# evroon/mav-detection

Measured on NVIDIA B200. Metric: 1080p frame-pairs/sec (flow+FoE+mask), higher is better.
Workload: dtype f32

## Files before the change

### include/mavd.h

```cpp
#ifndef MAVD_H_
#define MAVD_H_

#include <stddef.h>
#include <stdint.h>

#ifdef __cplusplus
extern "C" {
#endif

#define MAVD_ABI_VERSION 3

enum {
    MAVD_OK = 0,
    MAVD_ERR_INVALID = 1,
    MAVD_ERR_CUDA = 2,
    MAVD_ERR_UNSUPPORTED = 3,
    MAVD_ERR_NOMEM = 4
};

#define MAVD_FARNEBACK_GAUSSIAN 256

#define MAVD_N_SAMPLE_PAIRS 1000
#define MAVD_SAMPLES_PER_FRAME (4 * MAVD_N_SAMPLE_PAIRS)
#define MAVD_MAX_BOXES 32
// ... 14 lines not shown
    int32_t device;
    int32_t width;
    int32_t height;
    int32_t max_pairs;
    mavd_farneback_params farneback;
} mavd_config;

typedef struct mavd_imu {
    double ang[3];
    double dt;
    int32_t derotate;
    int32_t _pad;
} mavd_imu;

typedef struct mavd_detect_params {
    double magnitude_threshold;
    double ransac_threshold;
    double dyn_offset;
    double dyn_base;
    double dyn_gain;
    double dyn_min_mag;
    double fixed_min_mag;
    double fixed_angle;
} mavd_detect_params;

typedef struct mavd_tuning {
    int32_t mat_coord;
    int32_t pyr_staged;
    int32_t use_graph;
    int32_t polyexp_tma;
    int32_t iter_small_tiles;
    int32_t use_pdl;
    int32_t pyr_sweep;
    int32_t reserved[1];
} mavd_tuning;

typedef struct mavd_aux_inputs {
    const uint8_t* sky; int64_t sky_stride;
    const uint8_t* seg; int64_t seg_stride;
    const float* gt_flow;
} mavd_aux_inputs;

#define MAVD_HOST_BGR 1
#define MAVD_HOST_SEG_PACKED 2
#define MAVD_HOST_SKY_PACKED 4
#define MAVD_HOST_FIXED_PACKED 8
#define MAVD_HOST_COPY_ONLY 16

typedef struct mavd_frame_stats {
    double max_phi;
    int64_t n_total;
    int64_t n_fixed;
    int64_t positives;
    int64_t negatives;
    int64_t tp_total, fp_total;
    int64_t tp_fixed, fp_fixed;
    int32_t seg_bbox[4];
    double seg_flow_sum[2];
    double gt_flow_sum[2];
} mavd_frame_stats;

typedef struct mavd_frame_record {
    double foe[2];
    int32_t n_intersections;
    int32_t n_labels;
    mavd_frame_stats stats;
    int32_t boxes[MAVD_MAX_BOXES][5];
// ... 174 lines not shown
```

### mav_detection_b200/_lib.py

```python
from __future__ import annotations

import ctypes as C
import os
from typing import Optional

_HERE = os.path.dirname(os.path.abspath(__file__))
LIB_PATH = os.path.join(_HERE, 'csrc', 'libmavd.so')

ABI_VERSION = 3
MAVD_OK, MAVD_ERR_INVALID, MAVD_ERR_CUDA, MAVD_ERR_UNSUPPORTED, MAVD_ERR_NOMEM = 0, 1, 2, 3, 4
N_SAMPLE_PAIRS = 1000
SAMPLES_PER_FRAME = 4 * N_SAMPLE_PAIRS
MAX_BOXES = 32
HOST_SLOTS = 3
MAX_DETECTIONS = 256
OPTFLOW_FARNEBACK_GAUSSIAN = 256


class FarnebackParams(C.Structure):
    _fields_ = [('pyr_scale', C.c_double), ('levels', C.c_int32), ('winsize', C.c_int32),
                ('iterations', C.c_int32), ('poly_n', C.c_int32), ('poly_sigma', C.c_double),
                ('flags', C.c_int32)]


# ... 2 lines not shown
                ('max_pairs', C.c_int32), ('farneback', FarnebackParams)]


class Imu(C.Structure):
    _fields_ = [('ang', C.c_double * 3), ('dt', C.c_double), ('derotate', C.c_int32), ('_pad', C.c_int32)]


class DetectParams(C.Structure):
    _fields_ = [('magnitude_threshold', C.c_double), ('ransac_threshold', C.c_double),
                ('dyn_offset', C.c_double), ('dyn_base', C.c_double), ('dyn_gain', C.c_double),
                ('dyn_min_mag', C.c_double), ('fixed_min_mag', C.c_double), ('fixed_angle', C.c_double)]


class FrameStats(C.Structure):
    _fields_ = [('max_phi', C.c_double), ('n_total', C.c_int64), ('n_fixed', C.c_int64),
                ('positives', C.c_int64), ('negatives', C.c_int64), ('tp_total', C.c_int64),
                ('fp_total', C.c_int64), ('tp_fixed', C.c_int64), ('fp_fixed', C.c_int64),
                ('seg_bbox', C.c_int32 * 4), ('seg_flow_sum', C.c_double * 2), ('gt_flow_sum', C.c_double * 2)]


class FrameRecord(C.Structure):
    _fields_ = [('foe', C.c_double * 2), ('n_intersections', C.c_int32), ('n_labels', C.c_int32),
                ('stats', FrameStats), ('boxes', (C.c_int32 * 5) * MAX_BOXES)]


class Detection(C.Structure):
    _fields_ = [('label', C.c_int32), ('box', C.c_int32 * 4), ('area', C.c_int32), ('sum_x', C.c_int64),
                ('sum_y', C.c_int64), ('flow_sum', C.c_double * 2)]


class Tuning(C.Structure):
    _fields_ = [('mat_coord', C.c_int32), ('pyr_staged', C.c_int32), ('use_graph', C.c_int32),
                ('polyexp_tma', C.c_int32), ('iter_small_tiles', C.c_int32), ('use_pdl', C.c_int32),
                ('pyr_sweep', C.c_int32), ('reserved', C.c_int32 * 1)]


class AuxInputs(C.Structure):
    _fields_ = [('sky', C.c_void_p), ('sky_stride', C.c_int64), ('seg', C.c_void_p), ('seg_stride', C.c_int64),
                ('gt_flow', C.c_void_p)]


HOST_BGR, HOST_SEG_PACKED, HOST_SKY_PACKED, HOST_FIXED_PACKED, HOST_COPY_ONLY = 1, 2, 4, 8, 16

PROF_CLASSES = 12
PROF_NAMES = ['pyramid', 'polyexp', 'matrices', 'iter_full', 'iter_full_last', 'iter_coarse', 'foe', 'residual',
              'ccl']


class Profile(C.Structure):
    _fields_ = [('ms', C.c_double * PROF_CLASSES), ('launches', C.c_int64 * PROF_CLASSES)]


_P = C.c_void_p
SIGNATURES = {
    'mavd_abi_version': (C.c_int, []),
    'mavd_last_error': (C.c_char_p, []),
    'mavd_default_detect_params': (None, [C.POINTER(DetectParams)]),
    'mavd_create': (C.c_int, [C.POINTER(Config), C.POINTER(_P)]),
    'mavd_destroy': (C.c_int, [_P]),
    'mavd_workspace_bytes': (C.c_int, [_P, C.POINTER(C.c_size_t)]),
    'mavd_default_tuning': (None, [C.POINTER(Tuning)]),
    'mavd_set_tuning': (C.c_int, [_P, C.POINTER(Tuning)]),
    'mavd_get_tuning': (C.c_int, [_P, C.POINTER(Tuning)]),
    'mavd_level_info': (C.c_int, [_P, C.POINTER(C.c_int32), C.POINTER(C.c_int32), C.POINTER(C.c_int32)]),
    'mavd_bgr2gray': (C.c_int, [_P, _P, C.c_int64, _P]),
    'mavd_farneback': (C.c_int, [_P, _P, C.c_int32, C.c_int32, _P, _P]),
    'mavd_farneback_tap': (C.c_int, [_P, C.c_int32, C.c_int32, C.c_int32, _P, _P]),
# ... 91 lines not shown
```

### mav_detection_b200/csrc/api.cu

```cuda
#include <math.h>
#include <stdarg.h>
#include <stdlib.h>
#include <string.h>

#include <algorithm>
#include <new>
#include <vector>

#include "common.cuh"

namespace mavd {

static thread_local char g_err[512] = "";
std::atomic<int64_t> g_launches{0};

void set_error(const char* fmt, ...) {
    va_list ap;
    va_start(ap, fmt);
    vsnprintf(g_err, sizeof(g_err), fmt, ap);
    va_end(ap);
}

static inline int cv_round(double v) { return (int)nearbyint(v); }

// ... 431 lines not shown
    }
    H->bytes = A.bytes;
    cudaError_t e = cudaDeviceSynchronize();
    if (e != cudaSuccess) {
        set_error("device error during create: %s", cudaGetErrorString(e));
        return fail(MAVD_ERR_CUDA);
    }
    *out = H;
    return MAVD_OK;
#undef C_TRY
}

int mavd_destroy(mavd_handle h) {
    if (!h) return MAVD_OK;
    mavd_handle_full* H = static_cast<mavd_handle_full*>(h);
    DeviceGuard dg(H->cfg.device);
    cudaDeviceSynchronize();
    for (void* p : H->arena.ptrs) cudaFree(p);
    release_host_side(H);
    delete H;
    return MAVD_OK;
}

void mavd_default_tuning(mavd_tuning* t) {
    if (!t) return;
    memset(t, 0, sizeof(*t));
    t->mat_coord = 0;
    t->pyr_staged = 1;
    t->use_graph = 1;
    t->polyexp_tma = 1;
    t->iter_small_tiles = 1;
    t->use_pdl = 1;
    t->pyr_sweep = 1;
}

int mavd_set_tuning(mavd_handle h, const mavd_tuning* t) {
    MAVD_REQUIRE(h && t, MAVD_ERR_INVALID, "set_tuning: NULL argument");
    MAVD_REQUIRE(t->mat_coord >= 0 && t->mat_coord <= 2, MAVD_ERR_INVALID, "set_tuning: value out of range");
    DeviceGuard dg(h->cfg.device);
    MAVD_CUDA(cudaDeviceSynchronize());
    drop_graphs(h);
    h->tune = *t;
    return MAVD_OK;
}

int mavd_graph_stats(mavd_handle h, int32_t* n_captured, int32_t* n_direct) {
    MAVD_REQUIRE(h && n_captured && n_direct, MAVD_ERR_INVALID, "graph_stats: NULL argument");
    *n_captured = *n_direct = 0;
    for (const auto& g : h->graphs) ++*(g.exec ? n_captured : n_direct);
    return MAVD_OK;
}

int mavd_get_tuning(mavd_handle h, mavd_tuning* out) {
    MAVD_REQUIRE(h && out, MAVD_ERR_INVALID, "get_tuning: NULL argument");
    *out = h->tune;
    return MAVD_OK;
}

int mavd_profile_enable(mavd_handle h, int32_t on) {
    MAVD_REQUIRE(h != nullptr, MAVD_ERR_INVALID, "profile: handle is NULL");
    DeviceGuard dg(h->cfg.device);
    MAVD_CUDA(cudaDeviceSynchronize());
    for (auto& r : h->prof.recs) { h->prof.pool.push_back(r.a); h->prof.pool.push_back(r.b); }
    h->prof.recs.clear();
    h->prof.on = on != 0;
    return MAVD_OK;
// ... 807 lines not shown
```

### mav_detection_b200/csrc/farneback.cu

```cuda
#include <math.h>

#include "common.cuh"

namespace mavd {

__device__ __forceinline__ int reflect101(int i, int n) {
    while (i < 0 || i >= n) {
        if (n == 1) return 0;
        i = (i < 0) ? -i : 2 * (n - 1) - i;
    }
    return i;
}

__device__ __forceinline__ int clampi(int v, int lo, int hi) { return v < lo ? lo : (v > hi ? hi : v); }

struct PyrLevel {
    int w, h, pitch, taps;
    const int* xbase; const float* xtab;
    const float* xtabT;
    int staged;
    const int* ybase; const float* ytab;
    float* tmp; float* img;
    size_t tmp_stride, img_stride;
    int row0;
    int htiles_x;
};
struct PyrDesc {
    int n;
    PyrLevel lv[kMaxLevels];
};

__device__ __forceinline__ float byte_to_float(uint32_t v, uint32_t selector) {
    return __uint_as_float(__byte_perm(v, 0x4B000000u, selector)) - 8388608.f;
// ... 504 lines not shown
                    for (int k = 0; k < 4; ++k) {
                        const int gx = clampi(gx0 + k, 0, w - 1);
                        const int xm = reflect101(gx - 1, w), xp = reflect101(gx + 1, w);
                        const float h0 = 0.25f * q0[xm] + 0.5f * q0[gx] + 0.25f * q0[xp];
                        const float h1 = 0.25f * q1[xm] + 0.5f * q1[gx] + 0.25f * q1[xp];
                        const float h2 = 0.25f * q2[xm] + 0.5f * q2[gx] + 0.25f * q2[xp];
                        o[k] = 0.25f * h0 + 0.5f * h1 + 0.25f * h2;
                    }
                    v = make_float4(o[0], o[1], o[2], o[3]);
                }
                *reinterpret_cast<float4*>(&raw[(rr + PE_H - n) * PE_RW + 4 * g]) = v;
            }
        }
    }
    __syncthreads();
    polyexp_passes<N_>(raw, t, pc, n, tid, x0, y0, h, pitch, R + (size_t)blockIdx.z * 5 * plane, plane);
}

__device__ __forceinline__ void st_global_f32(float* p, float v) {
    asm volatile("st.global.f32 [%0], %1;" ::"l"(p), "f"(v));
}

__device__ __forceinline__ float border_factor(int d) { return d < 2 ? 0.14f : 0.4472f; }

struct R0Px { float y, x, yy, xx, xy; };

__device__ __forceinline__ R0Px load_r0_px(const float* __restrict__ R0, size_t o, size_t plane) {
    R0Px r;
    r.y = __ldg(R0 + o); r.x = __ldg(R0 + plane + o); r.yy = __ldg(R0 + 2 * plane + o);
    r.xx = __ldg(R0 + 3 * plane + o); r.xy = __ldg(R0 + 4 * plane + o);
    return r;
}

__device__ __forceinline__ void update_matrices_px(int x, int y, int w, int h, int pitch, size_t plane, float dx,
                                                   float dy, const R0Px& r0,
                                                   const float* __restrict__ R1, float* __restrict__ Mout) {
    const size_t o = (size_t)y * pitch + x;
    const float r0y = r0.y, r0x = r0.x, r0yy = r0.yy, r0xx = r0.xx, r0xy = r0.xy;
    float fx = (float)x + dx, fy = (float)y + dy;
    const float flx = floorf(fx), fly = floorf(fy);
    const int x1 = (int)fminf(fmaxf(flx, -2.f), 1.0e6f), y1 = (int)fminf(fmaxf(fly, -2.f), 1.0e6f);
    fx -= flx;
    fy -= fly;
    float r2, r3, r4, r5, r6;
    if ((unsigned)x1 < (unsigned)(w - 1) && (unsigned)y1 < (unsigned)(h - 1)) {
        const float a00 = (1.f - fx) * (1.f - fy), a01 = fx * (1.f - fy), a10 = (1.f - fx) * fy, a11 = fx * fy;
        const float* p = R1 + (size_t)y1 * pitch + x1;
        r2 = a00 * __ldg(p) + a01 * __ldg(p + 1) + a10 * __ldg(p + pitch) + a11 * __ldg(p + pitch + 1);
        p += plane;
        r3 = a00 * __ldg(p) + a01 * __ldg(p + 1) + a10 * __ldg(p + pitch) + a11 * __ldg(p + pitch + 1);
        p += plane;
        r4 = a00 * __ldg(p) + a01 * __ldg(p + 1) + a10 * __ldg(p + pitch) + a11 * __ldg(p + pitch + 1);
        p += plane;
        r5 = a00 * __ldg(p) + a01 * __ldg(p + 1) + a10 * __ldg(p + pitch) + a11 * __ldg(p + pitch + 1);
        p += plane;
        r6 = a00 * __ldg(p) + a01 * __ldg(p + 1) + a10 * __ldg(p + pitch) + a11 * __ldg(p + pitch + 1);
        r4 = (r0yy + r4) * 0.5f;
        r5 = (r0xx + r5) * 0.5f;
        r6 = (r0xy + r6) * 0.25f;
    } else {
        r2 = r3 = 0.f;
        r4 = r0yy;
        r5 = r0xx;
        r6 = r0xy * 0.5f;
    }
    r2 = (r0y - r2) * 0.5f;
    r3 = (r0x - r3) * 0.5f;
    r2 += r4 * dy + r6 * dx;
    r3 += r6 * dy + r5 * dx;
    if ((unsigned)(x - 5) >= (unsigned)(w - 10) || (unsigned)(y - 5) >= (unsigned)(h - 10)) {
        const float sc = (x < 5 ? border_factor(x) : 1.f) * (x >= w - 5 ? border_factor(w - x - 1) : 1.f) *
                         (y < 5 ? border_factor(y) : 1.f) * (y >= h - 5 ? border_factor(h - y - 1) : 1.f);
        r2 *= sc; r3 *= sc; r4 *= sc; r5 *= sc; r6 *= sc;
    }
    Mout[o] = r4 * r4 + r6 * r6;
    Mout[plane + o] = (r4 + r5) * r6;
    Mout[2 * plane + o] = r5 * r5 + r6 * r6;
    Mout[3 * plane + o] = r4 * r2 + r6 * r3;
    Mout[4 * plane + o] = r6 * r2 + r5 * r3;
}

__device__ __forceinline__ void resize_coord(int d, double scale, int src, int& i0, float& a) {
    const float f = (float)__dsub_rn(__dmul_rn(__dadd_rn((double)d, 0.5), scale), 0.5);
    int s = (int)floorf(f);
    a = f - (float)s;
    if (s < 0) { s = 0; a = 0.f; }
    if (s >= src - 1) { s = src - 1; a = 0.f; }
    i0 = s;
}

enum { MI_COORD_F64 = 0, MI_COORD_TABLES = 1, MI_COORD_POW2 = 2 };

__device__ __forceinline__ void resize_coord_pow2(int d, float scale, int src, int& i0, float& a) {
    const float f = __fsub_rn(__fmul_rn(__fadd_rn((float)d, 0.5f), scale), 0.5f);
    int s = (int)floorf(f);
    a = f - (float)s;
    if (s < 0) { s = 0; a = 0.f; }
    if (s >= src - 1) { s = src - 1; a = 0.f; }
    i0 = s;
}

constexpr int MI_TX = 64, MI_TY = 4;

template <int COORD>
__global__ void __launch_bounds__(256, 8) matrices_init_kernel(const float* __restrict__ R, size_t plane, int w, int h,
                                                           int pitch, size_t R_pair_stride,
                                                           const float2* __restrict__ cflow, int cw, int ch,
                                                           int cpitch, size_t cflow_stride,
                                                           const int* __restrict__ fxi0,
                                                           const float* __restrict__ fxa,
                                                           const int* __restrict__ fyi0,
                                                           const float* __restrict__ fya, float up_scale,
                                                           float* __restrict__ M, double xscale, double yscale, int r0_first) {
    pdl_entry();
    const int p = blockIdx.x;
    const int x = blockIdx.y * MI_TX + (threadIdx.x & (MI_TX - 1));
    const int y = blockIdx.z * MI_TY + threadIdx.x / MI_TX;
    if (x >= w || y >= h) return;
    const float* R0 = R + (size_t)p * R_pair_stride;
    R0Px r0;
    if (r0_first) r0 = load_r0_px(R0, (size_t)y * pitch + x, plane);
    float dx = 0.f, dy = 0.f;
    if (cflow) {
        const float2* cf = cflow + (size_t)p * cflow_stride;
        int xa0, ya0;
        float ax, ay;
        if (COORD == MI_COORD_TABLES) {
            xa0 = fxi0[x]; ya0 = fyi0[y]; ax = fxa[x]; ay = fya[y];
        } else if (COORD == MI_COORD_POW2) {
            resize_coord_pow2(x, (float)xscale, cw, xa0, ax);
            resize_coord_pow2(y, (float)yscale, ch, ya0, ay);
        } else {
            resize_coord(x, xscale, cw, xa0, ax);
            resize_coord(y, yscale, ch, ya0, ay);
        }
        const int xa1 = min(xa0 + 1, cw - 1), ya1 = min(ya0 + 1, ch - 1);
        const float2 f00 = cf[(size_t)ya0 * cpitch + xa0], f01 = cf[(size_t)ya0 * cpitch + xa1];
        const float2 f10 = cf[(size_t)ya1 * cpitch + xa0], f11 = cf[(size_t)ya1 * cpitch + xa1];
        const float tx0 = f00.x * (1.f - ax) + f01.x * ax, tx1 = f10.x * (1.f - ax) + f11.x * ax;
        const float ty0 = f00.y * (1.f - ax) + f01.y * ax, ty1 = f10.y * (1.f - ax) + f11.y * ax;
        dx = (tx0 * (1.f - ay) + tx1 * ay) * up_scale;
        dy = (ty0 * (1.f - ay) + ty1 * ay) * up_scale;
    }
    if (!r0_first) r0 = load_r0_px(R0, (size_t)y * pitch + x, plane);
    update_matrices_px(x, y, w, h, pitch, plane, dx, dy, r0, R0 + 5 * plane, M + (size_t)p * 5 * plane);
}

constexpr int IT_TX = 64, IT_TY = 32;
constexpr int IT_PAIR_GROUP = 4;

struct IterArgs {
    const float* Min;
    float* Mout;
    const float* R;
    float2* flow;
    int flow_pitch;
    size_t flow_stride;
    int w, h, pitch;
    size_t plane;
    int m;
    int hx;
    float scale;
    int pair_stride;
    const float* gk;
    int n_pairs, tiles_x;
};

template <int M_>
__device__ __forceinline__ void hsum_box(const float (&u)[20], float (&o)[4]) {
    float s = 0.f;
#pragma unroll
    for (int j = 8 - M_; j <= 8 + M_; ++j) s += u[j];
    o[0] = s;
#pragma unroll
    for (int j = 1; j < 4; ++j) {
        s += u[8 + M_ + j] - u[8 - M_ + j - 1];
        o[j] = s;
    }
}

template <int M_>
__device__ __forceinline__ void hsum_gauss(const float (&u)[20], const float* __restrict__ gk, float (&o)[4]) {
    float k[M_ + 1];
#pragma unroll
    for (int i = 0; i <= M_; ++i) k[i] = gk[i];
#pragma unroll
    for (int j = 0; j < 4; ++j) {
        float s = __fmul_rn(u[8 + j], k[0]);
#pragma unroll
        for (int i = 1; i <= M_; ++i) s = __fmaf_rn(u[8 + j - i] + u[8 + j + i], k[i], s);
        o[j] = s;
    }
}

template <int M_>
__device__ __forceinline__ void hsum_gauss_reg(const float (&u)[20], const float (&k)[M_ + 1], float (&o)[4]) {
#pragma unroll
    for (int j = 0; j < 4; ++j) {
// ... 297 lines not shown
                 a10 * __ldg(R1 + (q1 + plane)) + a11 * __ldg(R1 + (q1 + plane) + 1);
            r4 = a00 * __ldg(R1 + (q0 + 2 * plane)) + a01 * __ldg(R1 + (q0 + 2 * plane) + 1) +
                 a10 * __ldg(R1 + (q1 + 2 * plane)) + a11 * __ldg(R1 + (q1 + 2 * plane) + 1);
            r5 = a00 * __ldg(R1 + (q0 + 3 * plane)) + a01 * __ldg(R1 + (q0 + 3 * plane) + 1) +
                 a10 * __ldg(R1 + (q1 + 3 * plane)) + a11 * __ldg(R1 + (q1 + 3 * plane) + 1);
            r6 = a00 * __ldg(R1 + (q0 + 4 * plane)) + a01 * __ldg(R1 + (q0 + 4 * plane) + 1) +
                 a10 * __ldg(R1 + (q1 + 4 * plane)) + a11 * __ldg(R1 + (q1 + 4 * plane) + 1);
        }
        r4 = (r0yy + r4) * 0.5f;
        r5 = (r0xx + r5) * 0.5f;
        r6 = (r0xy + r6) * 0.25f;
    } else {
        r2 = r3 = 0.f;
        r4 = r0yy;
        r5 = r0xx;
        r6 = r0xy * 0.5f;
    }
    r2 = (r0y - r2) * 0.5f;
    r3 = (r0x - r3) * 0.5f;
    r2 += r4 * dy + r6 * dx;
    r3 += r6 * dy + r5 * dx;
    if (edge && ((unsigned)(x - 5) >= (unsigned)(w - 10) || (unsigned)(y - 5) >= (unsigned)(h - 10))) {
        const float sc = (x < 5 ? border_factor(x) : 1.f) * (x >= w - 5 ? border_factor(w - x - 1) : 1.f) *
                         (y < 5 ? border_factor(y) : 1.f) * (y >= h - 5 ? border_factor(h - y - 1) : 1.f);
        r2 *= sc; r3 *= sc; r4 *= sc; r5 *= sc; r6 *= sc;
    }
    st_global_f32(Mout + o, r4 * r4 + r6 * r6);
    st_global_f32(Mout + (o + plane), (r4 + r5) * r6);
    st_global_f32(Mout + (o + 2 * plane), r5 * r5 + r6 * r6);
    st_global_f32(Mout + (o + 3 * plane), r4 * r2 + r6 * r3);
    st_global_f32(Mout + (o + 4 * plane), r6 * r2 + r5 * r3);
}

template <int M_, bool LAST, int TY, bool GAUSS>
__global__ void __launch_bounds__(256, 3) iter_box_tma_kernel(const __grid_constant__ CUtensorMap tmap,
                                                              const __grid_constant__ CUtensorMap tmapR,
                                                              const __grid_constant__ CUtensorMap tmapRbox, IterArgs a) {
    pdl_entry();
    constexpr int NT = 256;
    constexpr int RW = IT_TX + 16;
    constexpr int RH = TY + 2 * M_;
    constexpr int CH = RH * RW;
    constexpr int NC = IT_TX + 2 * M_;
    constexpr int NW = NT / 32;
    extern __shared__ __align__(128) float box[];
    __shared__ __align__(8) uint64_t bar;
    const int tid = threadIdx.x, lane = tid & 31, warp = tid >> 5;
    const int n_tiles = gridDim.x / a.n_pairs;
    int p, tile;
    if (LAST) {
        p = blockIdx.x / n_tiles;
        tile = blockIdx.x - p * n_tiles;
    } else {
        const int per_group = IT_PAIR_GROUP * n_tiles;
        const int gidx = blockIdx.x / per_group, rem = blockIdx.x - gidx * per_group;
        const int gsize = min(IT_PAIR_GROUP, a.n_pairs - gidx * IT_PAIR_GROUP);
        tile = rem / gsize;
        p = gidx * IT_PAIR_GROUP + (rem - tile * gsize);
    }
    const int x0 = (tile % a.tiles_x) * IT_TX, y0 = (tile / a.tiles_x) * TY;
    const int w = a.w, h = a.h, pitch = a.pitch;
    const int plane = (int)a.plane;
    float gk[M_ + 1];
#pragma unroll
    for (int i = 0; i <= M_; ++i) gk[i] = GAUSS ? __ldg(a.gk + i) : 0.f;
    auto hsum = [&](const float (&u)[20], float (&o)[4]) {
        if (GAUSS) hsum_gauss_reg<M_>(u, gk, o);
        else hsum_box<M_>(u, o);
    };

    if (tid == 0) {
        mbar_init(&bar, 1);
        mbar_expect_tx(&bar, 5 * CH * (uint32_t)sizeof(float));
        tma_load_3d(box, &tmap, x0 - 8, y0 - M_, p * 5, &bar);
        if (!LAST) tma_prefetch_3d(&tmapR, x0 - 8, y0 - 8, p * a.pair_stride * 5);
    }
    const bool interior = (x0 - 8 >= 0) && (x0 + IT_TX + 8 <= w) && (y0 - M_ >= 0) && (y0 + TY + M_ <= h);
    __syncthreads();
    mbar_wait(&bar, 0);

    if (!interior) {
        const int xlo = max(0, 8 - x0), xhi = min(RW, w - x0 + 8);
        const int ylo = max(0, M_ - y0), yhi = min(RH, h - y0 + M_);
        const int ncol = xlo + (RW - xhi), nrow_in = yhi - ylo;
        if (ncol > 0) {
            const int per_plane = nrow_in * ncol;
            for (int idx = tid; idx < 5 * per_plane; idx += NT) {
                const int c = idx / per_plane, rem = idx - c * per_plane;
                const int rr = ylo + rem / ncol, k = rem % ncol;
                const int cc = k < xlo ? k : xhi + (k - xlo);
                float* row = box + c * CH + rr * RW;
                row[cc] = row[k < xlo ? xlo : xhi - 1];
            }
            __syncthreads();
        }
        const int nrow_out = ylo + (RH - yhi);
        if (nrow_out > 0) {
            const int per_plane = nrow_out * (RW / 4);
            for (int idx = tid; idx < 5 * per_plane; idx += NT) {
                const int c = idx / per_plane, rem = idx - c * per_plane;
                const int k = rem / (RW / 4), q = rem - k * (RW / 4);
                const int rr = k < ylo ? k : yhi + (k - ylo);
                float* pl = box + c * CH;
                reinterpret_cast<float4*>(pl + rr * RW)[q] = reinterpret_cast<const float4*>(pl + (k < ylo ? ylo : yhi - 1) * RW)[q];
            }
            __syncthreads();
        }
    }

    for (int t = warp; t < 15; t += NW) {
        const int c = t / 3, col = (t - 3 * c) * 32 + lane;
        if (col < NC) {
// ... 157 lines not shown
    R0Px cur = r0_of(0);
    mbar_wait(&bar, 1);
#pragma unroll
    for (int j = 0; j < PPT; ++j) {
        const int y = y0 + ((j * NT + tid) >> 6);
        R0Px nxt = cur;
        if (j + 1 < PPT) nxt = r0_of(j + 1);
        if (col_ok && y < h)
            update_matrices_box<RW, RH>(xp, y, w, h, pitch, (unsigned)plane, edge, ffx[j], ffy[j], cur, R1, Mout, box, bx, by);
        cur = nxt;
    }
}

__global__ void tap_planar_kernel(const float* __restrict__ src, int w, int h, int pitch, size_t plane, int nch,
                                  float* __restrict__ dst) {
    int x = blockIdx.x * blockDim.x + threadIdx.x, y = blockIdx.y;
    if (x >= w) return;
    for (int c = 0; c < nch; ++c) dst[((size_t)y * w + x) * nch + c] = src[c * plane + (size_t)y * pitch + x];
}
__global__ void tap_flow_kernel(const float2* __restrict__ src, int w, int h, int pitch, float2* __restrict__ dst) {
    int x = blockIdx.x * blockDim.x + threadIdx.x, y = blockIdx.y;
    if (x >= w) return;
    dst[(size_t)y * w + x] = src[(size_t)y * pitch + x];
}

template <bool GAUSS, bool LAST>
static int launch_iter(const IterArgs& a, dim3 grid, size_t smem, cudaStream_t s, bool pdl) {
    MAVD_CUDA((ensure_dynamic_smem<iter_kernel<GAUSS, LAST>>(200 * 1024)));
    MAVD_CUDA(launch_chained(pdl, iter_kernel<GAUSS, LAST>, grid, 256, smem, s, a));
    MAVD_LAUNCHED();
    return MAVD_OK;
}

template <int M_, bool LAST, int TY, bool GAUSS>
static int launch_iter_tma(const CUtensorMap& map, const CUtensorMap& mapR, const CUtensorMap& mapRbox, const IterArgs& a,
                           dim3 grid, cudaStream_t s, bool pdl) {
    constexpr size_t smem = sizeof(float) * 5 * (TY + 2 * M_) * (IT_TX + 16);
    MAVD_CUDA((ensure_dynamic_smem<iter_box_tma_kernel<M_, LAST, TY, GAUSS>>(smem)));
    MAVD_CUDA(launch_chained(pdl, iter_box_tma_kernel<M_, LAST, TY, GAUSS>, grid, 256, smem, s, map, mapR, mapRbox, a));
    MAVD_LAUNCHED();
    return MAVD_OK;
}

template <bool LAST>
static int launch_iter_tma_m(int m, bool gauss, bool small_tiles, const CUtensorMap& map, const CUtensorMap& mapR,
                             const CUtensorMap& mapRbox, const IterArgs& a, dim3 grid, cudaStream_t s, bool pdl) {
    using Launch = int (*)(const CUtensorMap&, const CUtensorMap&, const CUtensorMap&, const IterArgs&, dim3, cudaStream_t,
                           bool);
#define ITER_TMA_M(TY, GAUSS)                                                                                             \
    { launch_iter_tma<5, LAST, TY, GAUSS>, launch_iter_tma<6, LAST, TY, GAUSS>, launch_iter_tma<7, LAST, TY, GAUSS>,     \
      launch_iter_tma<8, LAST, TY, GAUSS> }
    static const Launch table[2][2][4] = {
        {ITER_TMA_M(IT_TY, false), ITER_TMA_M(16, false)},
        {ITER_TMA_M(IT_TY, true), ITER_TMA_M(16, true)}};
#undef ITER_TMA_M
    return table[gauss][small_tiles][m - 5](map, mapR, mapRbox, a, grid, s, pdl);
}

int farneback_run(mavd_handle H, const uint8_t* d_frames, int n_pairs, int pair_stride, float* d_flow,
                  cudaStream_t s) {
    const mavd_farneback_params& fp = H->cfg.farneback;
    const int W = H->cfg.width, Hh = H->cfg.height;
    const int n_frames = pair_stride == 1 ? n_pairs + 1 : 2 * n_pairs;
    const bool gauss = (fp.flags & MAVD_FARNEBACK_GAUSSIAN) != 0;
    const int m = fp.winsize / 2;
    const int hx = round_up(m, 4);
    const size_t frame_bytes = (size_t)W * Hh;

    auto lane = [&](cudaStream_t st) { return (st == H->s_aux && st != s) ? 1 : 0; };
    pdl_break(H, 0);
    pdl_break(H, 1);
    auto build_pyramid = [&](cudaStream_t st, int lo, int hi) -> int {
        if (H->n_levels <= 1 || lo > hi) return MAVD_OK;
        ProfScope ps(&H->prof, MAVD_PROF_PYRAMID, st);
        const int Wp = round_up(W, 4);
        const bool pyr_staged_env = H->tune.pyr_staged != 0;
        const int word_ok = ((W & 3) == 0 && (reinterpret_cast<uintptr_t>(d_frames) & 3) == 0) ? 1 : 0;
        auto make_desc = [&](int a, int b, PyrDesc& d, int& rows) {
            d.n = b - a + 1;
            rows = 0;
            for (int li = a; li <= b; ++li) {
                const Level& L = H->lv[li];
                PyrLevel& P = d.lv[li - a];
                P.w = L.w; P.h = L.h; P.pitch = L.pitch; P.taps = round_up(L.ksz + 1, 4);
                P.xbase = L.xbase; P.xtab = L.xtab; P.ybase = L.ybase; P.ytab = L.ytab;
                P.tmp = L.tmp; P.img = L.img; P.tmp_stride = (size_t)L.h * Wp; P.img_stride = L.plane;
                P.xtabT = L.xtabT;
// ... 106 lines not shown
            use_tma = (W % 16 == 0) && encode_tensor_map_3d(&tmap_u8, true, d_frames, (uint64_t)W, (uint64_t)Hh,
                                                            (uint64_t)n_frames, (uint64_t)W, (uint64_t)W * Hh, PE_BW,
                                                            (uint32_t)(PE_TY + 2 * H->poly.n + 2), 1u);
        else if (use_tma)
            use_tma = L.has_tmap_img;
        const bool pdl = pdl_next(H, lane(st));
#define PE_LAUNCH(N)                                                                                                   \
        do {                                                                                                           \
            if (li == 0 && use_tma)                                                                                    \
                MAVD_CUDA(launch_chained(pdl, polyexp_tma_kernel<true, N>, g, 256, 0, st, tmap_u8, L.w, L.h, L.pitch,   \
                                         H->poly, L.R, L.plane));                                                      \
            else if (li == 0)                                                                                          \
                MAVD_CUDA(launch_chained(pdl, polyexp_kernel<true, N>, g, 256, 0, st, (const void*)d_frames,            \
                                         frame_bytes, L.w, L.h, L.pitch, aligned, H->poly, L.R, L.plane));              \
            else if (use_tma)                                                                                          \
                MAVD_CUDA(launch_chained(pdl, polyexp_tma_kernel<false, N>, g, 256, 0, st, L.tmapImg, L.w, L.h,         \
                                         L.pitch, H->poly, L.R, L.plane));                                             \
            else                                                                                                       \
                MAVD_CUDA(launch_chained(pdl, polyexp_kernel<false, N>, g, 256, 0, st, (const void*)L.img, L.plane,     \
                                         L.w, L.h, L.pitch, 0, H->poly, L.R, L.plane));                                \
        } while (0)
        switch (H->poly.n) {
            case 5: PE_LAUNCH(5); break;
            case 7: PE_LAUNCH(7); break;
            case 8: PE_LAUNCH(8); break;
            default: PE_LAUNCH(0); break;
        }
#undef PE_LAUNCH
        MAVD_LAUNCHED();
        return MAVD_OK;
    };
    auto solve_level = [&](int li, cudaStream_t st) -> int {
        Level& L = H->lv[li];
        {
            ProfScope ps(&H->prof, MAVD_PROF_MATRICES, st);
            const bool top = (li == H->n_levels - 1);
            const Level* C = top ? nullptr : &H->lv[li + 1];
            const bool tables = H->tune.mat_coord == 1, no_pow2 = H->tune.mat_coord == 2;
            const double xscale = top ? 1.0 : 1.0 / ((double)L.w / C->w), yscale = top ? 1.0 : 1.0 / ((double)L.h / C->h);
            auto is_pow2 = [](double v) { int e; return v > 0.0 && frexp(v, &e) == 0.5 && e > -20 && e <= 1; };
            const int coord = tables ? MI_COORD_TABLES
                                     : (!no_pow2 && is_pow2(xscale) && is_pow2(yscale)) ? MI_COORD_POW2 : MI_COORD_F64;
            const dim3 g3(n_pairs, ceil_div(L.w, MI_TX), ceil_div(L.h, MI_TY));
#define MI_ARGS L.R, L.plane, L.w, L.h, L.pitch, (size_t)pair_stride * 5 * L.plane,                                     \
                top ? nullptr : (const float2*)C->flow, top ? 0 : C->w, top ? 0 : C->h, top ? 0 : C->pitch,             \
                top ? 0 : C->plane, L.fxi0, L.fxa, L.fyi0, L.fya, (float)(1.0 / fp.pyr_scale), L.M[0], xscale, yscale, 1
            const bool pdl = pdl_next(H, lane(st));
            if (coord == MI_COORD_TABLES) MAVD_CUDA(launch_chained(pdl, matrices_init_kernel<MI_COORD_TABLES>, g3, 256, 0, st, MI_ARGS));
            else if (coord == MI_COORD_POW2) MAVD_CUDA(launch_chained(pdl, matrices_init_kernel<MI_COORD_POW2>, g3, 256, 0, st, MI_ARGS));
            else MAVD_CUDA(launch_chained(pdl, matrices_init_kernel<MI_COORD_F64>, g3, 256, 0, st, MI_ARGS));
#undef MI_ARGS
            MAVD_LAUNCHED();
        }
        int cur = 0;
        for (int it = 0; it < fp.iterations; ++it) {
            const bool last = (it == fp.iterations - 1);
            IterArgs a;
            a.Min = L.M[cur];
            a.Mout = L.M[cur ^ 1];
            a.R = L.R;
            a.w = L.w; a.h = L.h; a.pitch = L.pitch; a.plane = L.plane;
            a.m = m; a.hx = hx;
            a.scale = gauss ? 1.f : (float)(1.0 / ((double)fp.winsize * fp.winsize));
            a.pair_stride = pair_stride;
            a.gk = gauss ? H->gauss_win : nullptr;
            if (last) {
                if (li == 0) {
                    a.flow = (float2*)d_flow; a.flow_pitch = W; a.flow_stride = (size_t)W * Hh;
                } else {
                    a.flow = (float2*)L.flow; a.flow_pitch = L.pitch; a.flow_stride = L.plane;
                }
            } else {
                a.flow = nullptr; a.flow_pitch = 0; a.flow_stride = 0;
            }
            dim3 g(ceil_div(L.w, IT_TX), ceil_div(L.h, IT_TY), n_pairs);
            a.n_pairs = n_pairs;
            a.tiles_x = g.x;
            const bool small_tiles =
                H->tune.iter_small_tiles != 0 && L.has_tmap16 && (long long)g.x * g.y * g.z <= 3LL * 148;
            const dim3 g1(small_tiles ? g.x * ceil_div(L.h, 16) * g.z : g.x * g.y * g.z);
            const int RW = IT_TX + 2 * hx, RH = IT_TY + 2 * m;
            const size_t smem = sizeof(float) * ((size_t)RH * RW + (size_t)IT_TY * RW + 5 * IT_TX * IT_TY);
            ProfScope ps(&H->prof, li > 0 ? MAVD_PROF_ITER_COARSE : (last ? MAVD_PROF_ITER_FULL_LAST : MAVD_PROF_ITER_FULL), st);
            int rc;
            const bool pdl = pdl_next(H, lane(st));
            if (m >= 5 && m <= 8 && L.has_tmap && !H->force_generic_iter) {
                const CUtensorMap& mM = small_tiles ? L.tmapM16[cur] : L.tmapM[cur];
                const CUtensorMap& mRb = small_tiles ? L.tmapRbox16 : L.tmapRbox;
                rc = last ? launch_iter_tma_m<true>(m, gauss, small_tiles, mM, L.tmapR, mRb, a, g1, st, pdl)
                          : launch_iter_tma_m<false>(m, gauss, small_tiles, mM, L.tmapR, mRb, a, g1, st, pdl);
            }
            else if (gauss) rc = last ? launch_iter<true, true>(a, g, smem, st, pdl) : launch_iter<true, false>(a, g, smem, st, pdl);
            else       rc = last ? launch_iter<false, true>(a, g, smem, st, pdl) : launch_iter<false, false>(a, g, smem, st, pdl);
            if (rc != MAVD_OK) return rc;
            if (!last) cur ^= 1;
        }
        L.last_m = cur;
        return MAVD_OK;
    };

    const bool fork = H->n_levels >= 3 && H->s_aux != nullptr;
    const int top_level = H->n_levels - 1;
    if (fork) {
        MAVD_CUDA(cudaEventRecord(H->ev_fork, s));
        MAVD_CUDA(cudaStreamWaitEvent(H->s_aux, H->ev_fork, 0));
        pdl_break(H, lane(H->s_aux));
        TRY_RC(build_pyramid(H->s_aux, 1, top_level));
        MAVD_CUDA(cudaEventRecord(H->ev_pyr, H->s_aux));
        for (int li = H->n_levels - 1; li >= 2; --li) {
            TRY_RC(expand_level(li, H->s_aux));
            TRY_RC(solve_level(li, H->s_aux));
        }
        MAVD_CUDA(cudaEventRecord(H->ev_join, H->s_aux));
        TRY_RC(expand_level(0, s));
        MAVD_CUDA(cudaStreamWaitEvent(s, H->ev_pyr, 0));
        pdl_break(H, lane(s));
        TRY_RC(expand_level(1, s));
        MAVD_CUDA(cudaStreamWaitEvent(s, H->ev_join, 0));
        pdl_break(H, lane(s));
        TRY_RC(solve_level(1, s));
        TRY_RC(solve_level(0, s));
    } else {
        TRY_RC(build_pyramid(s, 1, top_level));
// ... 52 lines not shown
```

Measured before the change: 5856.

## Fold Farneback matrix initialization into the first TMA iteration kernel

Adds a fused_init tuning option, on by default, that removes the separate matrices_init launch per pyramid level. The first non-last iteration kernel instead TMA-loads the R0 polynomial box, upsamples the coarse flow, bilinearly samples R1, and computes the initial M matrices into the shared halo in place. This drops a kernel launch and the full-plane write and re-read of M. In exchange, each tile redundantly recomputes matrices over its halo region and does extra scattered global gathers inside the iteration kernel.

Result: slower. 5535, median of 6 (-5.5%).

```diff
diff --git a/include/mavd.h b/include/mavd.h
--- a/include/mavd.h
+++ b/include/mavd.h
@@ -70,7 +70,7 @@
     int32_t iter_small_tiles;
     int32_t use_pdl;
     int32_t pyr_sweep;
-    int32_t reserved[1];
+    int32_t fused_init;
 } mavd_tuning;
 
 typedef struct mavd_aux_inputs {
diff --git a/mav_detection_b200/_lib.py b/mav_detection_b200/_lib.py
--- a/mav_detection_b200/_lib.py
+++ b/mav_detection_b200/_lib.py
@@ -58,7 +58,7 @@
 class Tuning(C.Structure):
     _fields_ = [('mat_coord', C.c_int32), ('pyr_staged', C.c_int32), ('use_graph', C.c_int32),
                 ('polyexp_tma', C.c_int32), ('iter_small_tiles', C.c_int32), ('use_pdl', C.c_int32),
-                ('pyr_sweep', C.c_int32), ('reserved', C.c_int32 * 1)]
+                ('pyr_sweep', C.c_int32), ('fused_init', C.c_int32)]
 
 
 class AuxInputs(C.Structure):
diff --git a/mav_detection_b200/csrc/api.cu b/mav_detection_b200/csrc/api.cu
--- a/mav_detection_b200/csrc/api.cu
+++ b/mav_detection_b200/csrc/api.cu
@@ -487,6 +487,7 @@
     t->iter_small_tiles = 1;
     t->use_pdl = 1;
     t->pyr_sweep = 1;
+    t->fused_init = 1;
 }
 
 int mavd_set_tuning(mavd_handle h, const mavd_tuning* t) {
diff --git a/mav_detection_b200/csrc/farneback.cu b/mav_detection_b200/csrc/farneback.cu
--- a/mav_detection_b200/csrc/farneback.cu
+++ b/mav_detection_b200/csrc/farneback.cu
@@ -1,4 +1,6 @@
 #include <math.h>
+
+#include <type_traits>
 
 #include "common.cuh"
 
@@ -569,20 +571,59 @@
     return r;
 }
 
+struct UmFootprint { int x1, y1; float a00, a01, a10, a11; bool inside; };
+
+__device__ __forceinline__ UmFootprint um_footprint(int x, int y, int w, int h, float dx, float dy) {
+    UmFootprint f;
+    float fx = (float)x + dx, fy = (float)y + dy;
+    const float flx = floorf(fx), fly = floorf(fy);
+    f.x1 = (int)fminf(fmaxf(flx, -2.f), 1.0e6f);
+    f.y1 = (int)fminf(fmaxf(fly, -2.f), 1.0e6f);
+    fx -= flx;
+    fy -= fly;
+    f.inside = (unsigned)f.x1 < (unsigned)(w - 1) && (unsigned)f.y1 < (unsigned)(h - 1);
+    f.a00 = (1.f - fx) * (1.f - fy); f.a01 = fx * (1.f - fy); f.a10 = (1.f - fx) * fy; f.a11 = fx * fy;
+    return f;
+}
+
+__device__ __forceinline__ void um_finish(int x, int y, int w, int h, float dx, float dy, const R0Px& r0, bool inside,
+                                          float r2, float r3, float r4, float r5, float r6, float (&mo)[5]) {
+    const float r0y = r0.y, r0x = r0.x, r0yy = r0.yy, r0xx = r0.xx, r0xy = r0.xy;
+    if (inside) {
+        r4 = (r0yy + r4) * 0.5f;
+        r5 = (r0xx + r5) * 0.5f;
+        r6 = (r0xy + r6) * 0.25f;
+    } else {
+        r2 = r3 = 0.f;
+        r4 = r0yy;
+        r5 = r0xx;
+        r6 = r0xy * 0.5f;
+    }
+    r2 = (r0y - r2) * 0.5f;
+    r3 = (r0x - r3) * 0.5f;
+    r2 += r4 * dy + r6 * dx;
+    r3 += r6 * dy + r5 * dx;
+    if ((unsigned)(x - 5) >= (unsigned)(w - 10) || (unsigned)(y - 5) >= (unsigned)(h - 10)) {
+        const float sc = (x < 5 ? border_factor(x) : 1.f) * (x >= w - 5 ? border_factor(w - x - 1) : 1.f) *
+                         (y < 5 ? border_factor(y) : 1.f) * (y >= h - 5 ? border_factor(h - y - 1) : 1.f);
+        r2 *= sc; r3 *= sc; r4 *= sc; r5 *= sc; r6 *= sc;
+    }
+    mo[0] = r4 * r4 + r6 * r6;
+    mo[1] = (r4 + r5) * r6;
+    mo[2] = r5 * r5 + r6 * r6;
+    mo[3] = r4 * r2 + r6 * r3;
+    mo[4] = r6 * r2 + r5 * r3;
+}
+
 __device__ __forceinline__ void update_matrices_px(int x, int y, int w, int h, int pitch, size_t plane, float dx,
                                                    float dy, const R0Px& r0,
                                                    const float* __restrict__ R1, float* __restrict__ Mout) {
     const size_t o = (size_t)y * pitch + x;
-    const float r0y = r0.y, r0x = r0.x, r0yy = r0.yy, r0xx = r0.xx, r0xy = r0.xy;
-    float fx = (float)x + dx, fy = (float)y + dy;
-    const float flx = floorf(fx), fly = floorf(fy);
-    const int x1 = (int)fminf(fmaxf(flx, -2.f), 1.0e6f), y1 = (int)fminf(fmaxf(fly, -2.f), 1.0e6f);
-    fx -= flx;
-    fy -= fly;
-    float r2, r3, r4, r5, r6;
-    if ((unsigned)x1 < (unsigned)(w - 1) && (unsigned)y1 < (unsigned)(h - 1)) {
-        const float a00 = (1.f - fx) * (1.f - fy), a01 = fx * (1.f - fy), a10 = (1.f - fx) * fy, a11 = fx * fy;
-        const float* p = R1 + (size_t)y1 * pitch + x1;
+    const UmFootprint f = um_footprint(x, y, w, h, dx, dy);
+    float r2 = 0.f, r3 = 0.f, r4 = 0.f, r5 = 0.f, r6 = 0.f;
+    if (f.inside) {
+        const float a00 = f.a00, a01 = f.a01, a10 = f.a10, a11 = f.a11;
+        const float* p = R1 + (size_t)f.y1 * pitch + f.x1;
         r2 = a00 * __ldg(p) + a01 * __ldg(p + 1) + a10 * __ldg(p + pitch) + a11 * __ldg(p + pitch + 1);
         p += plane;
         r3 = a00 * __ldg(p) + a01 * __ldg(p + 1) + a10 * __ldg(p + pitch) + a11 * __ldg(p + pitch + 1);
@@ -592,29 +633,14 @@
         r5 = a00 * __ldg(p) + a01 * __ldg(p + 1) + a10 * __ldg(p + pitch) + a11 * __ldg(p + pitch + 1);
         p += plane;
         r6 = a00 * __ldg(p) + a01 * __ldg(p + 1) + a10 * __ldg(p + pitch) + a11 * __ldg(p + pitch + 1);
-        r4 = (r0yy + r4) * 0.5f;
-        r5 = (r0xx + r5) * 0.5f;
-        r6 = (r0xy + r6) * 0.25f;
-    } else {
-        r2 = r3 = 0.f;
-        r4 = r0yy;
-        r5 = r0xx;
-        r6 = r0xy * 0.5f;
-    }
-    r2 = (r0y - r2) * 0.5f;
-    r3 = (r0x - r3) * 0.5f;
-    r2 += r4 * dy + r6 * dx;
-    r3 += r6 * dy + r5 * dx;
-    if ((unsigned)(x - 5) >= (unsigned)(w - 10) || (unsigned)(y - 5) >= (unsigned)(h - 10)) {
-        const float sc = (x < 5 ? border_factor(x) : 1.f) * (x >= w - 5 ? border_factor(w - x - 1) : 1.f) *
-                         (y < 5 ? border_factor(y) : 1.f) * (y >= h - 5 ? border_factor(h - y - 1) : 1.f);
-        r2 *= sc; r3 *= sc; r4 *= sc; r5 *= sc; r6 *= sc;
-    }
-    Mout[o] = r4 * r4 + r6 * r6;
-    Mout[plane + o] = (r4 + r5) * r6;
-    Mout[2 * plane + o] = r5 * r5 + r6 * r6;
-    Mout[3 * plane + o] = r4 * r2 + r6 * r3;
-    Mout[4 * plane + o] = r6 * r2 + r5 * r3;
+    }
+    float mo[5];
+    um_finish(x, y, w, h, dx, dy, r0, f.inside, r2, r3, r4, r5, r6, mo);
+    Mout[o] = mo[0];
+    Mout[plane + o] = mo[1];
+    Mout[2 * plane + o] = mo[2];
+    Mout[3 * plane + o] = mo[3];
+    Mout[4 * plane + o] = mo[4];
 }
 
 __device__ __forceinline__ void resize_coord(int d, double scale, int src, int& i0, float& a) {
@@ -635,6 +661,14 @@
     if (s < 0) { s = 0; a = 0.f; }
     if (s >= src - 1) { s = src - 1; a = 0.f; }
     i0 = s;
+}
+
+__device__ __forceinline__ void upsample_flow(float2 f00, float2 f01, float2 f10, float2 f11, float ax, float ay,
+                                              float up_scale, float& dx, float& dy) {
+    const float tx0 = f00.x * (1.f - ax) + f01.x * ax, tx1 = f10.x * (1.f - ax) + f11.x * ax;
+    const float ty0 = f00.y * (1.f - ax) + f01.y * ax, ty1 = f10.y * (1.f - ax) + f11.y * ax;
+    dx = (tx0 * (1.f - ay) + tx1 * ay) * up_scale;
+    dy = (ty0 * (1.f - ay) + ty1 * ay) * up_scale;
 }
 
 constexpr int MI_TX = 64, MI_TY = 4;
@@ -674,10 +708,7 @@
         const int xa1 = min(xa0 + 1, cw - 1), ya1 = min(ya0 + 1, ch - 1);
         const float2 f00 = cf[(size_t)ya0 * cpitch + xa0], f01 = cf[(size_t)ya0 * cpitch + xa1];
         const float2 f10 = cf[(size_t)ya1 * cpitch + xa0], f11 = cf[(size_t)ya1 * cpitch + xa1];
-        const float tx0 = f00.x * (1.f - ax) + f01.x * ax, tx1 = f10.x * (1.f - ax) + f11.x * ax;
-        const float ty0 = f00.y * (1.f - ax) + f01.y * ax, ty1 = f10.y * (1.f - ax) + f11.y * ax;
-        dx = (tx0 * (1.f - ay) + tx1 * ay) * up_scale;
-        dy = (ty0 * (1.f - ay) + ty1 * ay) * up_scale;
+        upsample_flow(f00, f01, f10, f11, ax, ay, up_scale, dx, dy);
     }
     if (!r0_first) r0 = load_r0_px(R0, (size_t)y * pitch + x, plane);
     update_matrices_px(x, y, w, h, pitch, plane, dx, dy, r0, R0 + 5 * plane, M + (size_t)p * 5 * plane);
@@ -701,6 +732,16 @@
     int pair_stride;
     const float* gk;
     int n_pairs, tiles_x;
+};
+
+struct IterInitArgs : IterArgs {
+    const float2* cflow;
+    int cw, ch, cpitch;
+    size_t cflow_stride;
+    int coord;
+    double xscale, yscale;
+    float up_scale;
+    const int* fxi0; const float* fxa; const int* fyi0; const float* fya;
 };
 
 template <int M_>
@@ -1064,11 +1105,13 @@
     st_global_f32(Mout + (o + 4 * plane), r6 * r2 + r5 * r3);
 }
 
-template <int M_, bool LAST, int TY, bool GAUSS>
+template <int M_, bool LAST, int TY, bool GAUSS, bool INIT = false>
 __global__ void __launch_bounds__(256, 3) iter_box_tma_kernel(const __grid_constant__ CUtensorMap tmap,
                                                               const __grid_constant__ CUtensorMap tmapR,
-                                                              const __grid_constant__ CUtensorMap tmapRbox, IterArgs a) {
+                                                              const __grid_constant__ CUtensorMap tmapRbox,
+                                                              std::conditional_t<INIT, IterInitArgs, IterArgs> a) {
     pdl_entry();
+    static_assert(!INIT || (!LAST && TY == IT_TY), "the level entry is folded into not-last 64 x 32 launches only");
     constexpr int NT = 256;
     constexpr int RW = IT_TX + 16;
     constexpr int RH = TY + 2 * M_;
@@ -1077,6 +1120,7 @@
     constexpr int NW = NT / 32;
     extern __shared__ __align__(128) float box[];
     __shared__ __align__(8) uint64_t bar;
+    __shared__ int4 s_col[INIT ? NC : 1], s_row[INIT ? RH : 1];
     const int tid = threadIdx.x, lane = tid & 31, warp = tid >> 5;
     const int n_tiles = gridDim.x / a.n_pairs;
     int p, tile;
@@ -1104,12 +1148,98 @@
     if (tid == 0) {
         mbar_init(&bar, 1);
         mbar_expect_tx(&bar, 5 * CH * (uint32_t)sizeof(float));
-        tma_load_3d(box, &tmap, x0 - 8, y0 - M_, p * 5, &bar);
+        if (INIT) tma_load_3d(box, &tmapRbox, x0 - 8, y0 - M_, p * a.pair_stride * 5, &bar);
+        else tma_load_3d(box, &tmap, x0 - 8, y0 - M_, p * 5, &bar);
         if (!LAST) tma_prefetch_3d(&tmapR, x0 - 8, y0 - 8, p * a.pair_stride * 5);
     }
     const bool interior = (x0 - 8 >= 0) && (x0 + IT_TX + 8 <= w) && (y0 - M_ >= 0) && (y0 + TY + M_ <= h);
+    if constexpr (INIT) {
+        if (a.cflow && tid < NC) {
+            const int x = clampi(x0 - M_ + tid, 0, w - 1);
+            int xa0;
+            float ax;
+            if (a.coord == MI_COORD_TABLES) { xa0 = a.fxi0[x]; ax = a.fxa[x]; }
+            else if (a.coord == MI_COORD_POW2) resize_coord_pow2(x, (float)a.xscale, a.cw, xa0, ax);
+            else resize_coord(x, a.xscale, a.cw, xa0, ax);
+            s_col[tid] = make_int4(x, xa0, min(xa0 + 1, a.cw - 1), __float_as_int(ax));
+        } else if (tid < NC) {
+            s_col[tid] = make_int4(clampi(x0 - M_ + tid, 0, w - 1), 0, 0, 0);
+        }
+        if (a.cflow && tid >= 128 && tid - 128 < RH) {
+            const int y = clampi(y0 - M_ + (tid - 128), 0, h - 1);
+            int ya0;
+            float ay;
+            if (a.coord == MI_COORD_TABLES) { ya0 = a.fyi0[y]; ay = a.fya[y]; }
+            else if (a.coord == MI_COORD_POW2) resize_coord_pow2(y, (float)a.yscale, a.ch, ya0, ay);
+            else resize_coord(y, a.yscale, a.ch, ya0, ay);
+            s_row[tid - 128] = make_int4(y, ya0 * a.cpitch, min(ya0 + 1, a.ch - 1) * a.cpitch, __float_as_int(ay));
+            int xs, xe;
+            float t;
+            const int bx0 = clampi(x0 - M_, 0, w - 1), bx1 = clampi(x0 + IT_TX + M_ - 1, 0, w - 1);
+            if (a.coord == MI_COORD_TABLES) { xs = a.fxi0[bx0]; xe = a.fxi0[bx1]; }
+            else if (a.coord == MI_COORD_POW2) {
+                resize_coord_pow2(bx0, (float)a.xscale, a.cw, xs, t);
+                resize_coord_pow2(bx1, (float)a.xscale, a.cw, xe, t);
+            } else {
+                resize_coord(bx0, a.xscale, a.cw, xs, t);
+                resize_coord(bx1, a.xscale, a.cw, xe, t);
+            }
+            xe = min(xe + 1, a.cw - 1);
+            const float2* cfr = a.cflow + (size_t)p * a.cflow_stride + (size_t)ya0 * a.cpitch;
+            const uintptr_t l0 = reinterpret_cast<uintptr_t>(cfr + xs) & ~(uintptr_t)127,
+                            l1 = reinterpret_cast<uintptr_t>(cfr + xe);
+            for (uintptr_t l = l0; l <= l1; l += 128) asm volatile("prefetch.global.L1 [%0];" ::"l"(l));
+        } else if (tid >= 128 && tid - 128 < RH) {
+            s_row[tid - 128] = make_int4(clampi(y0 - M_ + (tid - 128), 0, h - 1), 0, 0, 0);
+        }
+    }
     __syncthreads();
     mbar_wait(&bar, 0);
+
+    if constexpr (INIT) {
+        constexpr int NCELL = NC * RH;
+        const float2* cf = a.cflow ? a.cflow + (size_t)p * a.cflow_stride : nullptr;
+        const float* R1 = a.R + (size_t)(p * a.pair_stride + 1) * 5 * a.plane;
+        asm volatile("" : "+l"(R1));
+        const unsigned rstep = h > 1 ? (unsigned)pitch : 0u;
+#pragma unroll 1
+        for (int i0 = tid; i0 < NCELL; i0 += 2 * NT) {
+            float mo[2][5];
+            int cell[2];
+#pragma unroll
+            for (int k = 0; k < 2; ++k) {
+                const int i = min(i0 + k * NT, NCELL - 1);
+                const int rr = i / NC, cc = i - rr * NC;
+                cell[k] = rr * RW + (8 - M_) + cc;
+                const int4 col = s_col[cc], row = s_row[rr];
+                const int x = col.x, y = row.x;
+                const float* b = box + cell[k];
+                const R0Px r0{b[0], b[CH], b[2 * CH], b[3 * CH], b[4 * CH]};
+                float dx = 0.f, dy = 0.f;
+                if (cf) upsample_flow(cf[row.y + col.y], cf[row.y + col.z], cf[row.z + col.y], cf[row.z + col.z],
+                                      __int_as_float(col.w), __int_as_float(row.w), a.up_scale, dx, dy);
+                const UmFootprint f = um_footprint(x, y, w, h, dx, dy);
+                const unsigned q0 = (unsigned)(clampi(f.y1, 0, max(h - 2, 0)) * pitch + clampi(f.x1, 0, max(w - 2, 0)));
+                const unsigned q1 = q0 + rstep;
+                float s[5];
+#pragma unroll
+                for (int c = 0; c < 5; ++c) {
+                    const unsigned o = c * (unsigned)plane;
+                    s[c] = f.a00 * __ldg(R1 + (q0 + o)) + f.a01 * __ldg(R1 + (q0 + o) + 1) +
+                           f.a10 * __ldg(R1 + (q1 + o)) + f.a11 * __ldg(R1 + (q1 + o) + 1);
+                }
+                um_finish(x, y, w, h, dx, dy, r0, f.inside, s[0], s[1], s[2], s[3], s[4], mo[k]);
+                if (i0 + k * NT >= NCELL || x != x0 - M_ + cc || y != y0 - M_ + rr) cell[k] = -1;
+            }
+#pragma unroll
+            for (int k = 0; k < 2; ++k)
+                if (cell[k] >= 0) {
+#pragma unroll
+                    for (int c = 0; c < 5; ++c) box[c * CH + cell[k]] = mo[k][c];
+                }
+        }
+        __syncthreads();
+    }
 
     if (!interior) {
         const int xlo = max(0, 8 - x0), xhi = min(RW, w - x0 + 8);
@@ -1333,27 +1463,32 @@
     return MAVD_OK;
 }
 
-template <int M_, bool LAST, int TY, bool GAUSS>
-static int launch_iter_tma(const CUtensorMap& map, const CUtensorMap& mapR, const CUtensorMap& mapRbox, const IterArgs& a,
+template <int M_, bool LAST, int TY, bool GAUSS, bool INIT = false>
+static int launch_iter_tma(const CUtensorMap& map, const CUtensorMap& mapR, const CUtensorMap& mapRbox, const IterInitArgs& a,
                            dim3 grid, cudaStream_t s, bool pdl) {
     constexpr size_t smem = sizeof(float) * 5 * (TY + 2 * M_) * (IT_TX + 16);
-    MAVD_CUDA((ensure_dynamic_smem<iter_box_tma_kernel<M_, LAST, TY, GAUSS>>(smem)));
-    MAVD_CUDA(launch_chained(pdl, iter_box_tma_kernel<M_, LAST, TY, GAUSS>, grid, 256, smem, s, map, mapR, mapRbox, a));
+    MAVD_CUDA((ensure_dynamic_smem<iter_box_tma_kernel<M_, LAST, TY, GAUSS, INIT>>(smem)));
+    MAVD_CUDA(launch_chained(pdl, iter_box_tma_kernel<M_, LAST, TY, GAUSS, INIT>, grid, 256, smem, s, map, mapR, mapRbox, a));
     MAVD_LAUNCHED();
     return MAVD_OK;
 }
 
 template <bool LAST>
-static int launch_iter_tma_m(int m, bool gauss, bool small_tiles, const CUtensorMap& map, const CUtensorMap& mapR,
-                             const CUtensorMap& mapRbox, const IterArgs& a, dim3 grid, cudaStream_t s, bool pdl) {
-    using Launch = int (*)(const CUtensorMap&, const CUtensorMap&, const CUtensorMap&, const IterArgs&, dim3, cudaStream_t,
-                           bool);
-#define ITER_TMA_M(TY, GAUSS)                                                                                             \
-    { launch_iter_tma<5, LAST, TY, GAUSS>, launch_iter_tma<6, LAST, TY, GAUSS>, launch_iter_tma<7, LAST, TY, GAUSS>,     \
-      launch_iter_tma<8, LAST, TY, GAUSS> }
+static int launch_iter_tma_m(int m, bool gauss, bool small_tiles, bool init, const CUtensorMap& map,
+                             const CUtensorMap& mapR, const CUtensorMap& mapRbox, const IterInitArgs& a, dim3 grid,
+                             cudaStream_t s, bool pdl) {
+    using Launch = int (*)(const CUtensorMap&, const CUtensorMap&, const CUtensorMap&, const IterInitArgs&, dim3,
+                           cudaStream_t, bool);
+#define ITER_TMA_M(TY, GAUSS, INIT)                                                                                       \
+    { launch_iter_tma<5, LAST, TY, GAUSS, INIT>, launch_iter_tma<6, LAST, TY, GAUSS, INIT>,                             \
+      launch_iter_tma<7, LAST, TY, GAUSS, INIT>, launch_iter_tma<8, LAST, TY, GAUSS, INIT> }
+    if constexpr (!LAST) {
+        static const Launch init_table[2][4] = {ITER_TMA_M(IT_TY, false, true), ITER_TMA_M(IT_TY, true, true)};
+        if (init) return init_table[gauss][m - 5](map, mapR, mapRbox, a, grid, s, pdl);
+    }
     static const Launch table[2][2][4] = {
-        {ITER_TMA_M(IT_TY, false), ITER_TMA_M(16, false)},
-        {ITER_TMA_M(IT_TY, true), ITER_TMA_M(16, true)}};
+        {ITER_TMA_M(IT_TY, false, false), ITER_TMA_M(16, false, false)},
+        {ITER_TMA_M(IT_TY, true, false), ITER_TMA_M(16, true, false)}};
 #undef ITER_TMA_M
     return table[gauss][small_tiles][m - 5](map, mapR, mapRbox, a, grid, s, pdl);
 }
@@ -1526,15 +1661,20 @@
     };
     auto solve_level = [&](int li, cudaStream_t st) -> int {
         Level& L = H->lv[li];
-        {
+        const bool top = (li == H->n_levels - 1);
+        const Level* C = top ? nullptr : &H->lv[li + 1];
+        const bool tables = H->tune.mat_coord == 1, no_pow2 = H->tune.mat_coord == 2;
+        const double xscale = top ? 1.0 : 1.0 / ((double)L.w / C->w), yscale = top ? 1.0 : 1.0 / ((double)L.h / C->h);
+        auto is_pow2 = [](double v) { int e; return v > 0.0 && frexp(v, &e) == 0.5 && e > -20 && e <= 1; };
+        const int coord = tables ? MI_COORD_TABLES
+                                 : (!no_pow2 && is_pow2(xscale) && is_pow2(yscale)) ? MI_COORD_POW2 : MI_COORD_F64;
+        const dim3 g(ceil_div(L.w, IT_TX), ceil_div(L.h, IT_TY), n_pairs);
+        const bool tma_iter = m >= 5 && m <= 8 && L.has_tmap && !H->force_generic_iter;
+        const bool small_tiles =
+            H->tune.iter_small_tiles != 0 && L.has_tmap16 && (long long)g.x * g.y * g.z <= 3LL * 148;
+        const bool fused_init = (H->tune.fused_init == 1 || (H->tune.fused_init == 2 && li == 0)) && tma_iter && !small_tiles && fp.iterations >= 2;
+        if (!fused_init) {
             ProfScope ps(&H->prof, MAVD_PROF_MATRICES, st);
-            const bool top = (li == H->n_levels - 1);
-            const Level* C = top ? nullptr : &H->lv[li + 1];
-            const bool tables = H->tune.mat_coord == 1, no_pow2 = H->tune.mat_coord == 2;
-            const double xscale = top ? 1.0 : 1.0 / ((double)L.w / C->w), yscale = top ? 1.0 : 1.0 / ((double)L.h / C->h);
-            auto is_pow2 = [](double v) { int e; return v > 0.0 && frexp(v, &e) == 0.5 && e > -20 && e <= 1; };
-            const int coord = tables ? MI_COORD_TABLES
-                                     : (!no_pow2 && is_pow2(xscale) && is_pow2(yscale)) ? MI_COORD_POW2 : MI_COORD_F64;
             const dim3 g3(n_pairs, ceil_div(L.w, MI_TX), ceil_div(L.h, MI_TY));
 #define MI_ARGS L.R, L.plane, L.w, L.h, L.pitch, (size_t)pair_stride * 5 * L.plane,                                     \
                 top ? nullptr : (const float2*)C->flow, top ? 0 : C->w, top ? 0 : C->h, top ? 0 : C->pitch,             \
@@ -1549,7 +1689,7 @@
         int cur = 0;
         for (int it = 0; it < fp.iterations; ++it) {
             const bool last = (it == fp.iterations - 1);
-            IterArgs a;
+            IterInitArgs a;
             a.Min = L.M[cur];
             a.Mout = L.M[cur ^ 1];
             a.R = L.R;
@@ -1558,6 +1698,11 @@
             a.scale = gauss ? 1.f : (float)(1.0 / ((double)fp.winsize * fp.winsize));
             a.pair_stride = pair_stride;
             a.gk = gauss ? H->gauss_win : nullptr;
+            a.cflow = top ? nullptr : (const float2*)C->flow;
+            a.cw = top ? 0 : C->w; a.ch = top ? 0 : C->h; a.cpitch = top ? 0 : C->pitch;
+            a.cflow_stride = top ? 0 : C->plane;
+            a.coord = coord; a.xscale = xscale; a.yscale = yscale; a.up_scale = (float)(1.0 / fp.pyr_scale);
+            a.fxi0 = L.fxi0; a.fxa = L.fxa; a.fyi0 = L.fyi0; a.fya = L.fya;
             if (last) {
                 if (li == 0) {
                     a.flow = (float2*)d_flow; a.flow_pitch = W; a.flow_stride = (size_t)W * Hh;
@@ -1567,22 +1712,20 @@
             } else {
                 a.flow = nullptr; a.flow_pitch = 0; a.flow_stride = 0;
             }
-            dim3 g(ceil_div(L.w, IT_TX), ceil_div(L.h, IT_TY), n_pairs);
             a.n_pairs = n_pairs;
             a.tiles_x = g.x;
-            const bool small_tiles =
-                H->tune.iter_small_tiles != 0 && L.has_tmap16 && (long long)g.x * g.y * g.z <= 3LL * 148;
             const dim3 g1(small_tiles ? g.x * ceil_div(L.h, 16) * g.z : g.x * g.y * g.z);
             const int RW = IT_TX + 2 * hx, RH = IT_TY + 2 * m;
             const size_t smem = sizeof(float) * ((size_t)RH * RW + (size_t)IT_TY * RW + 5 * IT_TX * IT_TY);
             ProfScope ps(&H->prof, li > 0 ? MAVD_PROF_ITER_COARSE : (last ? MAVD_PROF_ITER_FULL_LAST : MAVD_PROF_ITER_FULL), st);
             int rc;
             const bool pdl = pdl_next(H, lane(st));
-            if (m >= 5 && m <= 8 && L.has_tmap && !H->force_generic_iter) {
+            if (tma_iter) {
                 const CUtensorMap& mM = small_tiles ? L.tmapM16[cur] : L.tmapM[cur];
                 const CUtensorMap& mRb = small_tiles ? L.tmapRbox16 : L.tmapRbox;
-                rc = last ? launch_iter_tma_m<true>(m, gauss, small_tiles, mM, L.tmapR, mRb, a, g1, st, pdl)
-                          : launch_iter_tma_m<false>(m, gauss, small_tiles, mM, L.tmapR, mRb, a, g1, st, pdl);
+                const bool init = fused_init && it == 0;
+                rc = last ? launch_iter_tma_m<true>(m, gauss, small_tiles, false, mM, L.tmapR, mRb, a, g1, st, pdl)
+                          : launch_iter_tma_m<false>(m, gauss, small_tiles, init, mM, L.tmapR, mRb, a, g1, st, pdl);
             }
             else if (gauss) rc = last ? launch_iter<true, true>(a, g, smem, st, pdl) : launch_iter<true, false>(a, g, smem, st, pdl);
             else       rc = last ? launch_iter<false, true>(a, g, smem, st, pdl) : launch_iter<false, false>(a, g, smem, st, pdl);
```
